# pypr/pysph

Hardware: AMD Instinct MI355X
Metric: particle-updates/sec (nnps.update + AccelerationEval.compute), WCSPH 3D, fp64 (higher is better)
Workload: dtype f64

## Files before the change

include/sphhip.h:

```cpp
#ifndef SPHHIP_H
#define SPHHIP_H

#include <stddef.h>
#include <stdint.h>

#ifdef __cplusplus
extern "C" {
#endif

#define SPH_MAX_ARRAYS 8
#define SPH_MAX_PAR 16
#define SPH_MAX_EQS 64

typedef struct sph_ctx sph_ctx;

enum sph_status {
    SPH_OK = 0,
    SPH_ERR_HIP = -1,
    SPH_ERR_ARG = -2,
    SPH_ERR_CELLS = -3,
    SPH_ERR_UNSUPPORTED = -4,
    SPH_ERR_MISSING_PROP = -5,
    SPH_ERR_STATE = -6
};
// ... 215 lines not shown
int sph_domain_counts_queue(sph_ctx *ctx);
int sph_domain_counts_collect(sph_ctx *ctx, double *out);
int sph_array_h_known(sph_ctx *ctx, int array_id, double *hmin, double *hmax);
int sph_array_props(sph_ctx *ctx, int array_id, int *out, int cap, int *n);
int sph_coord_histogram(sph_ctx *ctx, int array_id, int axis, double vmin, double span, int nbins, uint32_t *host_out);

enum sph_stepper {
    SPH_STEP_WCSPH = 1,
    SPH_STEP_TVF = 2,
    SPH_STEP_SOLID_MECH = 3
};
int sph_integrate_stage(sph_ctx *ctx, int array_id, int stepper, int stage, double dt);
int sph_reduce_min(sph_ctx *ctx, int array_id, int prop, double *out);

int sph_set_option(sph_ctx *ctx, const char *key, long value);

int sph_timer_enable(sph_ctx *ctx, int on);
int sph_timer_reset(sph_ctx *ctx);
int sph_timer_get(sph_ctx *ctx, const char *key, double *ms, long *count);

long sph_abi_sizeof(const char *struct_name);
long sph_abi_offsetof(const char *struct_name, const char *field);

#ifdef __cplusplus
}
#endif
#endif
```

pysph_amd/csrc/sph_eval.hip:

```cpp
#include "sph_internal.h"
#include "sph_kernels.h"
#include "sph_pair.h"

#include <cfloat>
#include <cmath>
#include <type_traits>

struct EosArgs {
    int kind;
    double par[SPH_MAX_PAR];
    double *rho, *p, *cs;
    size_t start, stop;
    double *q[SPH_PROP_COUNT];
    uint32_t *tflag;
};

__device__ inline void jacobi_eigen3(double A[3][3], double V[3][3], double d[3])
{
    for (int i = 0; i < 3; i++) for (int j = 0; j < 3; j++) V[i][j] = (i == j) ? 1.0 : 0.0;
    for (int sweep = 0; sweep < 12; sweep++) {
        double off = fabs(A[0][1]) + fabs(A[0][2]) + fabs(A[1][2]);
        double diag = fabs(A[0][0]) + fabs(A[1][1]) + fabs(A[2][2]);
        if (off <= 1e-300 || off <= 1e-18 * diag) break;
#pragma unroll
// ... 455 lines not shown
        if (a.dflags & F_MOM) {
            T au = D.au + a.p.gx, av = D.av + a.p.gy, aw = D.aw + a.p.gz;
            a.p.au[o] = au; a.p.av[o] = av; a.p.aw[o] = aw;
            a.p.dt_cfl[o] = D.dt_cfl < T(0.0) ? T(0.0) : D.dt_cfl + a.p.c0;
            a.p.dt_force[o] = au * au + av * av + aw * aw;
        }
        if (a.dflags & F_XSPH) {
            a.p.ax[o] = D.ax + D.u; a.p.ay[o] = D.ay + D.v; a.p.az[o] = D.az + D.w;
        }
    }
};
typedef FamWCSPH_T<double> FamWCSPH;

template <class T, bool UM = false> struct FamWCSPHE_T : FamWCSPH_T<T> {
    static constexpr bool EOSF = true;
    static constexpr bool UMASS = UM;
    static constexpr int NR = 8;
    struct Raw {
        typename std::conditional<sizeof(T) == 8, double2, float4>::type q[sizeof(T) == 8 ? 4 : 2];
    };
    template <class A> static __device__ __forceinline__ void load_raw(const A &a, uint32_t jg, Raw &r)
    {
        if constexpr (sizeof(T) == 8) {
            const double2 *p = reinterpret_cast<const double2 *>(a.rec) + (unsigned long long)jg * 4;
            r.q[0] = p[0]; r.q[1] = p[1]; r.q[2] = p[2]; r.q[3] = p[3];
        } else {
            const float4 *p = reinterpret_cast<const float4 *>(a.rec) + (unsigned long long)jg * 2;
            r.q[0] = p[0]; r.q[1] = p[1];
        }
    }
    template <class A> static __device__ __forceinline__ void decode(const A &a, const Raw &r, uint32_t fl, T mu, real4<T> &pj, T (&s)[8],
                                                                     int gk = 3)
    {
        T rho;
        if constexpr (sizeof(T) == 8) {
            pj.x = r.q[0].x; pj.y = r.q[0].y; pj.z = r.q[1].x; pj.w = 0.0;
            s[0] = r.q[1].y; s[1] = r.q[2].x; s[2] = r.q[2].y; s[3] = r.q[3].y; rho = r.q[3].x;
        } else {
            pj.x = r.q[0].x; pj.y = r.q[0].y; pj.z = r.q[0].z; pj.w = 0.f;
            s[0] = r.q[0].w; s[1] = r.q[1].x; s[2] = r.q[1].y; s[3] = r.q[1].w; rho = r.q[1].z;
        }
        s[4] = rho;
        s[5] = s[6] = s[7] = T(0.0);
        if constexpr (UM) {
            const T q = s[3];
            s[3] = mu;
            if (fl & F_MOM) {
                const T ratio = rho * (T)a.e_rho01;
                s[5] = q;
                s[6] = (T)a.e_c0 * tait_cs_power(ratio, gk);
// ... 14 lines not shown
        Raw r;
        load_raw(a, jg, r);
        decode(a, r, fl, mu, pj, s);
    }
};

template <class T, bool UM = false> struct FamWCSPHEG_T : FamWCSPHE_T<T, UM> {
    typedef FamWCSPHE_T<T, UM> Base;
    template <class A> static __device__ __forceinline__ void load_fused(const A &a, uint32_t jg, uint32_t fl, T mu, real4<T> &pj, T (&s)[8])
    {
        typename Base::Raw r;
        Base::load_raw(a, jg, r);
        Base::decode(a, r, fl, mu, pj, s, a.e_gk);
    }
};

template <class T> struct FamWCSPHV_T : FamWCSPH_T<T> {
    static constexpr bool EOSF = true;
    static constexpr int NR = 8;
    template <class A> static __device__ __forceinline__ void load_fused(const A &a, uint32_t jg, uint32_t fl, T mu, real4<T> &pj, T (&s)[8])
    {
        T rho;
        if constexpr (sizeof(T) == 8) {
            const double2 *p = reinterpret_cast<const double2 *>(a.rec) + (unsigned long long)jg * 4;
            const double2 q0 = p[0], q1 = p[1], q2 = p[2], q3 = p[3];
            pj.x = q0.x; pj.y = q0.y; pj.z = q1.x; pj.w = q1.y;
            s[0] = q2.x; s[1] = q2.y; s[2] = q3.x; rho = q3.y;
        } else {
            const float4 *p = reinterpret_cast<const float4 *>(a.rec) + (unsigned long long)jg * 2;
            const float4 q0 = p[0], q1 = p[1];
            pj.x = q0.x; pj.y = q0.y; pj.z = q0.z; pj.w = q0.w;
            s[0] = q1.x; s[1] = q1.y; s[2] = q1.z; rho = q1.w;
        }
        s[3] = mu;
        s[4] = rho;
        s[5] = s[6] = s[7] = T(0.0);
        if (fl & F_MOM) {
            const T ratio = rho * (T)a.e_rho01;
            T r7, r3;
            tait_powers(ratio, 3, r7, r3);
            const T p = (T)a.e_p0 + (T)a.e_B * (r7 - T(1.0));
            s[5] = rho != T(0.0) ? p * fast_rcp(rho * rho) : T(0.0);
            s[6] = (T)a.e_c0 * r3;
            s[7] = p;
        }
    }
};

#define WCSPHM_CT(f00, f01, f10, f11) ((uint32_t)(f00) | ((uint32_t)(f01) << 4) | ((uint32_t)(f10) << 8) | ((uint32_t)(f11) << 12))
template <class T> struct FamWCSPHM_T : FamWCSPHE_T<T, true> {
    typedef FamWCSPHE_T<T, true> Base;
    typedef typename Base::Raw Raw;
// ... 85 lines not shown
        const uint32_t ct = a.dflags;
        const uint32_t row = D.dc ? ((ct >> 8) | (ct >> 12)) & 15u : (ct | (ct >> 4)) & 15u;
        const size_t base = __builtin_offsetof(A, p) + __builtin_offsetof(Params, out) + (size_t)slot * (9 * sizeof(double *));
        auto out = [&](int k) { return kernarg_read<double *>(base + (size_t)k * sizeof(double *)); };
        if (row & F_CONT) out(0)[o] = D.arho;
        if (row & F_MOM) {
            const T au = D.au + a.p.gx, av = D.av + a.p.gy, aw = D.aw + a.p.gz;
            out(1)[o] = au; out(2)[o] = av; out(3)[o] = aw;
            out(7)[o] = D.dt_cfl < T(0.0) ? T(0.0) : D.dt_cfl + a.p.c0;
            out(8)[o] = au * au + av * av + aw * aw;
        }
        if (row & F_XSPH) {
            out(4)[o] = D.ax + D.u; out(5)[o] = D.ay + D.v; out(6)[o] = D.az + D.w;
        }
    }
};

template <class T> struct FamWCSPHMV_T : FamWCSPHM_T<T> {
    typedef FamWCSPHM_T<T> Base;
    template <class A> static __device__ __forceinline__ void load_fused(const A &a, uint32_t jg, uint32_t, T mu, real4<T> &pj, T (&s)[8])
    {
        T rho;
        if constexpr (sizeof(T) == 8) {
            const double2 *p = reinterpret_cast<const double2 *>(a.rec) + (unsigned long long)jg * 4;
            const double2 q0 = p[0], q1 = p[1], q2 = p[2], q3 = p[3];
            pj.x = q0.x; pj.y = q0.y; pj.z = q1.x; pj.w = q1.y;
            s[0] = q2.x; s[1] = q2.y; s[2] = q3.x; rho = q3.y;
        } else {
            const float4 *p = reinterpret_cast<const float4 *>(a.rec) + (unsigned long long)jg * 2;
            const float4 q0 = p[0], q1 = p[1];
            pj.x = q0.x; pj.y = q0.y; pj.z = q0.z; pj.w = q0.w;
            s[0] = q1.x; s[1] = q1.y; s[2] = q1.z; rho = q1.w;
        }
        const bool c1 = rho < T(0.0);
        s[3] = c1 ? -(T)a.p.mu1 : mu;
        rho = fabs(rho);
        s[4] = rho;
        const T ratio = rho * (T)a.e_rho01;
        T r7, r3;
        tait_powers(ratio, 3, r7, r3);
        const T p = (T)a.e_p0 + (T)a.e_B * (r7 - T(1.0));
        s[5] = rho != T(0.0) ? p * fast_rcp(rho * rho) : T(0.0);
        s[6] = (T)a.e_c0 * r3;
        s[7] = T(0.0);
    }
};

template <bool UH>
__device__ __forceinline__ void load_record_wcsph(const double *__restrict__ rj, uint32_t fl, double4 &pj, double (&s)[8])
{
    const double2 *r2 = reinterpret_cast<const double2 *>(rj);
    const double2 a0 = r2[0], a1 = r2[1], b0 = r2[2], b1 = r2[3], c = r2[4];
// ... 163 lines not shown
typedef FamTVF_T<double> FamTVF;

template <> __device__ __forceinline__ void load_record<FamTVF, true>(const double *__restrict__ rj, uint32_t fl, double4 &pj, double (&s)[12])
{
    const double2 *r2 = reinterpret_cast<const double2 *>(rj);
    const double2 a0 = r2[0], a1 = r2[1], b0 = r2[2], b1 = r2[3], c0 = r2[4];
    pj.x = a0.x; pj.y = a0.y; pj.z = a1.x; pj.w = 0.0;
    s[0] = b0.x; s[1] = b0.y; s[2] = b1.x; s[6] = a1.y; s[7] = b1.y; s[8] = 0.0; s[9] = 0.0; s[10] = c0.x; s[11] = 0.0;
    s[3] = s[4] = 0.0; s[5] = c0.y;
    if (fl & F_TAS) {
        const double2 d0 = r2[5];
        s[3] = d0.x; s[4] = d0.y;
    }
    if (fl & F_TAV) s[9] = r2[6].x;
}

template <class T> struct FamTVFE_T : FamTVF_T<T> {
    static constexpr bool EOSF = true;
    static constexpr int NA = 12;
    template <class A> static __device__ __forceinline__ void load_fused(const A &a, uint32_t jg, uint32_t fl, T mu, real4<T> &pj, T (&s)[12])
    {
        T rho;
        if constexpr (sizeof(T) == 8) {
            const double2 *p = reinterpret_cast<const double2 *>(a.rec) + (unsigned long long)jg * (unsigned)(a.nrec >> 1);
            const double2 q0 = p[0], q1 = p[1], q2 = p[2], q3 = p[3];
            pj.x = q0.x; pj.y = q0.y; pj.z = q1.x; pj.w = 0.0; rho = q1.y;
            s[0] = q2.x; s[1] = q2.y; s[2] = q3.x; s[3] = q3.y; s[4] = s[5] = 0.0;
            if (fl & F_TAS) { const double2 q4 = p[4]; s[4] = q4.x; s[5] = q4.y; }
        } else {
            const float4 *p = reinterpret_cast<const float4 *>(a.rec) + (unsigned long long)jg * (unsigned)(a.nrec >> 2);
            const float4 q0 = p[0], q1 = p[1];
            pj.x = q0.x; pj.y = q0.y; pj.z = q0.z; pj.w = 0.f; rho = q0.w;
            s[0] = q1.x; s[1] = q1.y; s[2] = q1.z; s[3] = q1.w; s[4] = s[5] = 0.f;
            if (fl & F_TAS) { const float4 q2 = p[2]; s[4] = q2.x; s[5] = q2.y; }
        }
        s[6] = rho;
        s[7] = (T)a.e_p0 * (rho * (T)a.e_rho01 - (T)a.e_B);
        s[8] = T(0.0);
        s[9] = mu;
        const T vj = mu * fast_rcp(rho);
        s[10] = vj * vj;
        s[11] = T(0.0);
    }
};

template <class T> struct FamVGrad_T {
    typedef T Real;
    static constexpr bool PRED = true;
    static constexpr uint32_t CF0 = F_VG3;
    static constexpr int MINB = 4;
    static constexpr int NA = 4;
    static constexpr int NR = 8;
    struct Params { double *v[9]; };
// ... 143 lines not shown
#pragma unroll
            for (int k = 0; k < 7; k++) q[k] = p[k];
            if (with_r) { q[7] = p[7]; q[8] = p[8]; q[9] = p[9]; }
            else q[7] = q[8] = q[9] = make_double2(0.0, 0.0);
            pj.x = q[0].x; pj.y = q[0].y; pj.z = q[1].x; pj.w = 0.0;
            s[0] = q[1].y; s[1] = q[2].x; s[2] = q[2].y; s[3] = mu; s[4] = q[3].x; s[5] = q[3].y;
#pragma unroll
            for (int k = 0; k < 6; k++) { s[6 + 2 * k] = q[4 + k].x; s[7 + 2 * k] = q[4 + k].y; }
        } else {
            float4 q[5];
#pragma unroll
            for (int k = 0; k < 4; k++) q[k] = p[k];
            if (with_r) q[4] = p[4];
            else { q[4] = make_float4(0.f, 0.f, 0.f, 0.f); q[3].z = 0.f; q[3].w = 0.f; }
            pj.x = q[0].x; pj.y = q[0].y; pj.z = q[0].z; pj.w = 0.f;
            s[0] = q[0].w; s[1] = q[1].x; s[2] = q[1].y; s[3] = mu; s[4] = q[1].z; s[5] = q[1].w;
#pragma unroll
            for (int k = 0; k < 3; k++) { s[6 + 4 * k] = q[2 + k].x; s[7 + 4 * k] = q[2 + k].y; s[8 + 4 * k] = q[2 + k].z; s[9 + 4 * k] = q[2 + k].w; }
        }
    }
    template <class A> static __device__ __forceinline__ void load_fused(const A &a, uint32_t jg, uint32_t, T mu, real4<T> &pj, T (&s)[18],
                                                                         uint32_t with_r = 1u)
    {
        decode(reinterpret_cast<const Piece *>(a.rec) + (unsigned long long)jg * PIECES, mu, pj, s, with_r);
    }
};

template <class Fam> __device__ __forceinline__ void load_aux(double (&s)[Fam::NA], const double *__restrict__ p)
{
#pragma unroll
    for (int k = 0; k < Fam::NA; k++) s[k] = p[k];
}

template <class Fam, int KK, bool UH> __global__ __launch_bounds__(256) void k_pair_direct(PairArgs<Fam> a)
{
    uint32_t i = blockIdx.x * blockDim.x + threadIdx.x;
    if (i >= a.nd) return;
    uint32_t o = a.d_perm[i];
    if (o < a.d_start || o >= a.d_stop) return;
    double4 pi = a.posh[a.d_off + i];
    typename Fam::Dest D;
    Fam::load(D, a.aux + (size_t)(a.d_off + i) * Fam::NA, a, o);
    uint32_t key = a.d_keys[i];
    int cx = key % a.nc[0];
    int t = key / a.nc[0];
    int cy = t % a.nc[1], cz = t / a.nc[1];
    double hi2 = a.radius_scale * pi.w;
// ... 166 lines not shown
        if (prop == SPH_M || prop == SPH_U || prop == SPH_V || prop == SPH_W) return true;
        if (prop == SPH_RHO) return flags & (F_MOM | F_XSPH);
        if (prop == SPH_P || prop == SPH_CS) return flags & F_MOM;
        return false;
    }
    if (fam == FAM_DENSITY) return prop == SPH_M;
    if (fam == FAM_NBR) return false;
    if (fam == FAM_VGRAD) return true;
    if (fam == FAM_ELASTIC) {
        if (prop == SPH_U || prop == SPH_V || prop == SPH_W || prop == SPH_M) return true;
        if (prop == SPH_RHO) return flags & (F_ESTRESS | F_EAV | F_EXSPH);
        if (prop == SPH_CS) return flags & F_EAV;
        if (prop == SPH_P) return flags & F_ESTRESS;
        if (prop >= SPH_S00 && prop <= SPH_S22) return flags & F_ESTRESS;
        return false;
    }
    if (fam == FAM_TVF) {
        if (prop == SPH_UHAT || prop == SPH_VHAT || prop == SPH_WHAT) return flags & F_TAS;
        return true;
    }
    return false;
}

static int pack_pieces(const PackArgs &pa)
{
    if (!pa.rec) return 0;
    if (pa.layout == 6) return 4;
    if (pa.layout == 7) return 2;
    if (pa.layout == 8) return pa.nr / 2;
    if (pa.layout == 9) return pa.nr / 4;
    if (pa.layout == 10) return 10;
    if (pa.layout == 11) return 5;
    if (pa.layout == 12) return 4;
    if (pa.layout == 13) return 2;
    if (pa.layout == 5) return (pa.nr % 4) ? 0 : pa.nr / 4;
    if (pa.nr % 2) return 0;
    return pa.nr / 2;
}

static void launch_pack(sph_ctx *c, const PackArgs &pa, size_t n)
{
    const dim3 g(div_up(n, 256)), b(256);
    const size_t lds = (size_t)pa.lds_np * 256 * 16;
    switch (pa.rec ? pa.layout : -1) {
    case 2: hipLaunchKernelGGL(k_pack<2>, g, b, lds, c->stream, pa); break;
    case 3: hipLaunchKernelGGL(k_pack<3>, g, b, lds, c->stream, pa); break;
// ... 207 lines not shown
    return SPH_OK;
}

int nnps_csr_pair_kernel(sph_ctx *c, int src, int dst, uint32_t *count, const uint32_t *start, uint32_t *nbrs)
{
    SPH_TRY(nnps_need_tables(c));
    DevArray &S = c->arr[src], &D = c->arr[dst];
    if (D.n == 0) return SPH_OK;
    if (count && D.n > D.n_binned) HIP_TRY(hipMemsetAsync(count + D.n_binned, 0, (D.n - D.n_binned) * 4, c->stream));
    const bool uh = c->uniform_h && c->use_uniform_h;
    const bool dest_is_src = src == dst;
    const size_t total = S.n + (dest_is_src ? 0 : D.n);
    if (total >= (1ull << 32)) { sph_set_error("too many particles for 32-bit packed indices"); return SPH_ERR_ARG; }
    PackPlan pl = pack_plan(FAM_NBR);
    if (uh) pl.nr = 4;
    const bool was_f32 = c->record_f32 != 0, was_a32 = c->arith_f32 != 0;
    c->record_f32 = 0; c->arith_f32 = 0;
    c->cur_eosf = false;
    c->cur_eosv = false;
    c->cur_tvff = false;
    c->cur_elu = false;
    c->cur_umass = false;
    c->cur_nrec = pl.nr;
    int rc = c->posh.reserve((total + 64) * sizeof(double) * pl.nr);
    if (rc == SPH_OK) rc = c->aux.reserve(64);
    if (rc == SPH_OK) rc = c->fposb.reserve((total + 64) * sizeof(float4));
    for (auto &pc : c->pack_cache) pc.epoch = 0;
    if (rc == SPH_OK) rc = pack_array(c, src, 0, pl, FAM_NBR, 1u, false, true, 0);
    if (rc == SPH_OK && S.g_n > 0) rc = pack_array(c, src, 0, pl, FAM_NBR, 1u, false, true, 1);
    if (rc == SPH_OK && !dest_is_src) rc = pack_array(c, dst, S.n, pl, FAM_NBR, 1u, true, true, 0);
    c->record_f32 = was_f32; c->arith_f32 = was_a32;
    if (rc != SPH_OK) return rc;
    sph_kernel K;
    K.kind = 1; K.dim = c->dim; K.fac = 1.0; K.radius_scale = c->radius_scale; K.deltap = 0.0;
    PairArgs<FamNbr> a;
    memset(&a, 0, sizeof a);
    fill_common(c, a, &K, 0.0);
    a.ablate = 0; a.dbg = nullptr;
    a.nsrc = 1;
    a.src[0] = {S.cell_start.as<uint32_t>(), 0u, 1u, S.fine_start.as<uint32_t>(), 0.0, 0u};
    if (S.g_n > 0) a.src[a.nsrc++] = {S.g_cell_start.as<uint32_t>(), (uint32_t)S.n_binned, 1u, S.g_fine_start.as<uint32_t>(), 0.0, 1u};
    a.d_off = dest_is_src ? 0u : (uint32_t)S.n;
    a.nd = (uint32_t)D.n_binned;
    a.d_keys = D.keys_sorted.as<uint32_t>(); a.d_fkeys = D.fkeys_sorted.as<uint32_t>(); a.d_perm = D.perm.as<uint32_t>();
    set_tile_order(c, a, D);
    a.d_start = 0; a.d_stop = (uint32_t)D.n; a.dflags = 1u;
    a.p.count = count; a.p.start = start; a.p.nbrs = nbrs;
// ... 82 lines not shown
        if (!A.m_known) return SPH_OK;
        if (have[cls[a]] && mu[cls[a]] != A.m_value) return SPH_OK;
        mu[cls[a]] = A.m_value; have[cls[a]] = true;
    }
    DevArray &M = c->merged;
    if (M.n == 0) { *done = true; return SPH_OK; }

    static const int outp[9] = {SPH_ARHO, SPH_AU, SPH_AV, SPH_AW, SPH_AX, SPH_AY, SPH_AZ, SPH_DT_CFL, SPH_DT_FORCE};
    static const int inp[9] = {SPH_X, SPH_Y, SPH_Z, SPH_U, SPH_V, SPH_W, SPH_RHO, SPH_P, SPH_H};
    const bool f32 = c->arith_f32 != 0;
    PackMArgs pa;
    memset(&pa, 0, sizeof pa);
    for (int a = 0; a < na; a++) {
        const int id = c->ids[a];
        DevArray &A = c->arr[id];
        for (int k = 0; k < 9; k++) {
            if (A.n && !A.prop[inp[k]]) return need_prop(c, id, inp[k], "pair loop");
            pa.prop[k][a] = A.prop[inp[k]];
        }
        if (cls[a]) pa.cls |= 1u << a;
    }
    c->cur_eosf = !vh; c->cur_umass = !vh; c->cur_tvff = false; c->cur_elu = false; c->cur_eosv = vh;
    c->cur_nrec = 8;
    SPH_TRY(c->posh.reserve((M.n + 64) * (f32 ? 32 : 64)));
    SPH_TRY(c->aux.reserve(64));
    SPH_TRY(c->fposb.reserve((M.n + 64) * sizeof(float4)));
    for (auto &pc : c->pack_cache) pc.epoch = 0;
    {
        ScopedTimer tm(c, T_PACK);
        pa.perm = M.perm.as<uint32_t>(); pa.slot = M.slot8.as<uint8_t>();
        pa.n = M.n; pa.off = 0;
        pa.rec = c->posh.as<double>(); pa.fpos = c->fposb.as<float4>();
        pa.f32 = f32 ? 1 : 0; pa.lds_np = f32 ? 2 : 4;
        for (int k = 0; k < 3; k++) pa.gmin[k] = c->xmin[k];
        pa.vh = vh ? 1 : 0;
        pa.hr = vh ? c->radius_scale : c->radius_scale * c->h_uniform;
        pa.rho_flag = c->xflag.as<uint32_t>();
        const dim3 pg(div_up(M.n, 256)), pb(256);
        const size_t plds = (size_t)pa.lds_np * 256 * 16;
        if (f32 && vh) hipLaunchKernelGGL((k_pack_merged<true, true>), pg, pb, plds, c->stream, pa);
        else if (f32) hipLaunchKernelGGL((k_pack_merged<true, false>), pg, pb, plds, c->stream, pa);
        else if (vh) hipLaunchKernelGGL((k_pack_merged<false, true>), pg, pb, plds, c->stream, pa);
        else hipLaunchKernelGGL((k_pack_merged<false, false>), pg, pb, plds, c->stream, pa);
    }
    ScopedTimer tm(c, T_PAIR);
    ScopedTimer tmf(c, T_PAIR_FAM + FAM_WCSPH);
// ... 199 lines not shown
                    !(c->uniform_h && c->use_uniform_h) && !(dflags & F_TENSILE) && tait_gk(g->eos_par[2]) == 3 && g->eos_par[0] > 0.0 &&
                    !c->record_f32 && !c->wcsph_nr;
        if (eosv) c->want_mrange = true;
        for (int j = 0; j < nsrcs && eosv; j++) eosv = c->arr[srcs[j]].m_known;
        if (eosv) pl.nr = 8;
        c->cur_eosv = eosv;
        bool tvff = g->src_eos == 2 && c->eos_fuse && c->mass_fuse && fam == FAM_TVF && c->pair_variant == 6 && c->uniform_h &&
                    c->use_uniform_h && !c->record_f32 && g->eos_par[1] != 0.0;
        if (tvff) c->want_mrange = true;
        for (int j = 0; j < nsrcs && tvff; j++) tvff = c->arr[srcs[j]].m_known;
        if (tvff && !dest_is_src) tvff = D.m_known;
        if (tvff) pl.nr = c->arith_f32 ? ((dflags & F_TAS) ? 12 : 8) : ((dflags & F_TAS) ? 10 : 8);
        bool elu = fam == FAM_ELASTIC && c->mass_fuse && c->pair_variant == 6 && c->uniform_h && c->use_uniform_h && !c->record_f32;
        if (elu) c->want_mrange = true;
        for (int j = 0; j < nsrcs && elu; j++) elu = c->arr[srcs[j]].m_known;
        if (elu) pl.nr = 20;
        c->cur_elu = elu;
        c->cur_tvff = tvff;
        c->cur_umass = umass;
        c->cur_eosf = eosf;
        c->cur_nrec = pl.nr;
        const void *rec_was = c->posh.ptr, *fpos_was = c->fposb.ptr;
        const size_t total_res = phase == 1 ? std::max(total, D.cap) : total;
        SPH_TRY(c->posh.reserve((total_res + 64) * sizeof(double) * (c->pair_variant >= 2 ? pl.nr : 4), phase == 2, c->stream));
        SPH_TRY(c->aux.reserve((total_res + 64) * sizeof(double) * pl.na));
        if (c->pair_variant >= 3) SPH_TRY(c->fposb.reserve((total_res + 64) * sizeof(float4), phase == 2, c->stream));
        if (c->posh.ptr != rec_was || c->fposb.ptr != fpos_was)
            for (auto &pc : c->pack_cache) pc.epoch = 0;
        {
            ScopedTimer tm(c, T_PACK);
            const int sig = pl.nr * 32 + (c->record_f32 ? 1 : 0) + (c->arith_f32 ? 2 : 0) + (eosf ? 4 : 0) + (umass ? 8 : 0) + (tvff || elu || eosv ? 16 : 0);
            if (phase == 1) c->phase_sig = sig;
            const bool repack = phase == 2 && c->phase_sig != sig;
            bool keep = share;
            if (share)
                for (auto &pc : c->pack_cache)
                    if (pc.epoch == c->pack_epoch && (pc.fam != fam || pc.sig != sig)) keep = false;
            if (!keep)
                for (auto &pc : c->pack_cache) pc.epoch = 0;
            auto pack_once = [&](int id, size_t off, uint32_t fl, bool dest_only) -> int {
                PackCache &pc = c->pack_cache[id];
                const bool hit = share && pc.epoch == c->pack_epoch && pc.fam == fam && pc.sig == sig;
                if (phase != 2 || repack) SPH_TRY(pack_array(c, id, off, pl, fam, fl, dest_only, !hit, 0));
                if (phase != 1 && c->arr[id].g_n > 0) SPH_TRY(pack_array(c, id, off, pl, fam, fl, dest_only, !hit, 1));
                pc.epoch = share ? c->pack_epoch : 0; pc.fam = fam; pc.sig = sig;
                return SPH_OK;
// ... 324 lines not shown
            if (D.nnps_slot < 0) { sph_set_error("destination array %d is not part of the neighbour grid", dst); return SPH_ERR_STATE; }
            if (c->ghosts_binned) { sph_set_error("generated families do not read ghost segments (ghost split): use the plain exchange -> sph_nnps_update order"); return SPH_ERR_UNSUPPORTED; }
            SPH_TRY(nnps_need_tables(c));
            size_t total = 0, off_of[SPH_MAX_ARRAYS];
            bool dest_is_src = false;
            for (int jj = 0; jj < ns; jj++) {
                const int s = f->src[idx[jj]];
                if (c->arr[s].nnps_slot < 0) { sph_set_error("source array %d is not part of the neighbour grid", s); return SPH_ERR_STATE; }
                off_of[jj] = total; total += c->arr[s].n; dest_is_src |= s == dst;
            }
            size_t d_off = total;
            if (!dest_is_src) total += D.n;
            else for (int jj = 0; jj < ns; jj++) if (f->src[idx[jj]] == dst) d_off = off_of[jj];
            if (total >= (1ull << 32)) { sph_set_error("too many particles for 32-bit packed indices"); return SPH_ERR_ARG; }
            const int na = f->n_sprops;
            const bool compact = q.uniform_h != 0;
            const int na_fam = ((na + 1) & ~1) < 2 ? 2 : ((na + 1) & ~1);
            a32 = c->arith_f32 && f->launch_f32 != nullptr;
            const bool rf32 = c->record_f32 || a32;
            const int nr = rf32 ? ((4 + na_fam + 3) & ~3)
                         : compact ? ((3 + na + 1) & ~1) : 4 + ((na + 1) & ~1);
            const int layout = rf32 ? 5 : (compact ? 4 : 0);
            q.rec_f32 = rf32 ? 1 : 0;
            SPH_TRY(c->posh.reserve((total + 64) * sizeof(double) * nr));
            for (auto &pc : c->pack_cache) pc.epoch = 0;
            SPH_TRY(c->aux.reserve(64));
            SPH_TRY(c->fposb.reserve((total + 64) * sizeof(float4)));
            {
                ScopedTimer tm(c, T_PACK);
                for (int jj = 0; jj < ns; jj++) SPH_TRY(pack_generic(c, f->src[idx[jj]], off_of[jj], na, f->sprops, nr, layout));
                if (!dest_is_src) {
                    int have[SPH_GEN_MAX_SPROPS], nh = 0;
                    for (int k = 0; k < na; k++) if (D.prop[f->sprops[k]]) have[nh++] = f->sprops[k];
                    SPH_TRY(pack_generic(c, dst, d_off, nh == na ? na : 0, f->sprops, nr, layout));
                }
            }
            q.rec = c->posh.as<double>();
            q.nrec = nr;
            q.fpos = c->fposb.as<float4>();
            q.dom_extent = fmax(fmax(c->xmax[0] - c->xmin[0], c->xmax[1] - c->xmin[1]), c->xmax[2] - c->xmin[2]);
            for (int k = 0; k < 3; k++) { q.nc[k] = c->nc[k]; q.xmin[k] = c->xmin[k]; }
            q.cell_size = c->cell_size;
            q.radius_scale = c->radius_scale;
            q.hu = 0.5 * (c->h_uniform + c->h_uniform);
            q.h1u = 1.0 / q.hu;
            q.facu = K->fac * q.h1u;
// ... 90 lines not shown
```

pysph_amd/csrc/sph_pair.h:

```cpp
#pragma once

#include <hip/hip_runtime.h>
#include <cstdint>

#include "sphhip.h"
#include "sph_kernels.h"

template <class T> __device__ __forceinline__ T r2_exact(T dx, T dy, T dz)
{
#pragma clang fp contract(off)
    const T a = dx * dx, b = dy * dy, c = dz * dz;
    return (a + b) + c;
}

template <class T> struct Real4Of;
template <> struct Real4Of<double> { typedef double4 type; };
template <> struct Real4Of<float> { typedef float4 type; };
template <class T> using real4 = typename Real4Of<T>::type;


struct KernelConst {
    double sigma;
    double deltap;
    int dim;
// ... 173 lines not shown
    T gg = aa * y, hh = 0.5 * y;
    const T rr = fma(-hh, gg, 0.5);
    hh = fma(hh, rr, hh);
    const T t = hh + hh;
    g.rinv = t * P;
    g.rij = r2c * g.rinv;
    g.q = g.rij * g.h1;
    return t * g.rij;
}

template <int KK, bool UH, class T> __device__ __forceinline__ T pair_w(const PairGeomT<T> &g) { return SphKernel<KK>::template w<UH>(g.q) * g.fac; }
template <int KK, bool UH, class T> __device__ __forceinline__ T pair_gradh(const PairGeomT<T> &g, int dim)
{
    return -g.fac * g.h1 * (SphKernel<KK>::template dw<UH>(g.q) * g.q + SphKernel<KK>::template w<UH>(g.q) * (T)dim);
}
template <int KK, bool UH, class T> __device__ __forceinline__ T pair_gradfac(const PairGeomT<T> &g)
{
    T t;
    if (SphKernel<KK>::HAS_DWQ) t = SphKernel<KK>::template dwq<UH>(g.q) * (g.fac * g.h1 * g.h1);
    else t = SphKernel<KK>::template dw<UH>(g.q) * (g.fac * g.h1) * g.rinv;
    return g.rij > T(1e-12) ? t : T(0);
}

template <class Fam, bool UH>
__device__ __forceinline__ void load_record(const double *__restrict__ rj, uint32_t fl, double4 &pj, double (&s)[Fam::NA])
{
    pj = *reinterpret_cast<const double4 *>(rj);
#pragma unroll
    for (int k = 0; k < Fam::NA; k++) s[k] = rj[4 + k];
}

template <class Fam, class T>
__device__ __forceinline__ void load_record_f32(const float *__restrict__ rj, real4<T> &pj, T (&s)[Fam::NA])
{
    constexpr int NF = (4 + Fam::NA + 3) & ~3;
    float f[NF];
    const float4 *r4 = reinterpret_cast<const float4 *>(rj);
#pragma unroll
    for (int q = 0; q < NF / 4; q++) { const float4 t = r4[q]; f[4 * q] = t.x; f[4 * q + 1] = t.y; f[4 * q + 2] = t.z; f[4 * q + 3] = t.w; }
    pj.x = f[0]; pj.y = f[1]; pj.z = f[2]; pj.w = f[3];
#pragma unroll
    for (int k = 0; k < Fam::NA; k++) s[k] = f[4 + k];
}

template <int NA, class T>
__device__ __forceinline__ void pin_record(const real4<T> &pj, const T (&s)[NA])
// ... 38 lines not shown
#endif
#define WLQ SPH_WLQ
#define WCAP_UH SPH_WCAP_UH
#define WCAP_VH 136
#define WCSL 96
#define NLW (64 * (1 + 3 * WLQ))
#define NL_NONE 0xFFFFFFFFu
#define XWIN (SPH_NSUB + 1)

#ifndef WPB
#define WPB 1
#endif

template <class Fam, int KK, bool UH, bool F32 = false, uint32_t CF = 0>
__global__ __launch_bounds__(64 * WPB, Fam::MINB) void k_pair_wave(PairArgs<Fam> a)
{
    typedef typename Fam::Real T;
    static_assert(F32 || sizeof(T) == 8, "fp32 arithmetic reads fp32 records");
    const uint32_t NR = (uint32_t)a.nrec;
    constexpr int WCAP = UH ? WCAP_UH : WCAP_VH;
    constexpr int TS = WCAP + 8;
    __shared__ __attribute__((aligned(16))) float tile_[WPB][(UH ? 3 : 4) * TS];
    __shared__ unsigned short csl_[WPB][WCSL];
    __shared__ unsigned long long smask_[WPB][WLQ][64];
    __shared__ uint32_t sjb_[WPB][WLQ][64];
    const int wv = __builtin_amdgcn_readfirstlane((int)(threadIdx.x >> 6));
    float *const tile = tile_[wv];
    float *const tx = tile, *const ty = tile + TS, *const tz = tile + 2 * TS, *const tw = tile + (UH ? 0 : 3 * TS);
    unsigned short *const csl = csl_[wv];
    unsigned long long (*const smask)[64] = smask_[wv];
    uint32_t (*const sjb)[64] = sjb_[wv];

    const int t = threadIdx.x & 63;
    const uint32_t wt = xcd_tile(blockIdx.x, gridDim.x) * WPB + (uint32_t)wv;
    uint32_t dtile = wt >> 2;
    if (dtile * 256u >= a.nd) return;
    if (a.d_tile_order) dtile = a.d_tile_order[dtile];
    const uint32_t tbase = dtile * 256u + (wt & 3u) * 64u;
    const uint32_t i = tbase + t;
    if (tbase >= a.nd) return;
    const bool valid = i < a.nd;
    uint32_t ic = valid ? i : a.nd - 1;
    if (a.d_list) ic = a.d_list[ic];
    const uint32_t o = a.d_perm[ic];
    uint32_t slot = 0;
    bool active;
    if constexpr (fam_merged<Fam>::value) {
        slot = a.d_slot[ic];
        const unsigned long long rg = kernarg_read<unsigned long long>(__builtin_offsetof(PairArgs<Fam>, p) + Fam::rng_offset(slot));
        active = valid && o >= (uint32_t)rg && o < (uint32_t)(rg >> 32);
    } else {
        active = valid && o >= a.d_start && o < a.d_stop;
    }
    const uint32_t fkey = a.d_fkeys[ic];
    const uint32_t key = fkey / SPH_NSUB;
    const int ncx = a.nc[0], ncy = a.nc[1], ncz = a.nc[2];
    const int row = key / ncx;
    const int cx = (int)(key % ncx) * SPH_NSUB + (int)(fkey % SPH_NSUB);
    bool facew = true;
    if (a.face_mode != 0 || a.gfx_lo > -0x7fffffff || a.gfx_hi < 0x7fffffff) {
        int mn = active ? cx : 0x7fffffff, mx = active ? cx : -0x7fffffff;
#pragma unroll
        for (int o = 32; o > 0; o >>= 1) { mn = min(mn, __shfl_xor(mn, o, 64)); mx = max(mx, __shfl_xor(mx, o, 64)); }
        mn = __builtin_amdgcn_readfirstlane(mn); mx = __builtin_amdgcn_readfirstlane(mx);
        facew = mn <= mx && (mn - XWIN <= a.gfx_lo || mx + XWIN >= a.gfx_hi);
        if (mn > mx && !a.nl_mode) return;
        if (a.face_mode == 1 && facew) return;
        if (a.face_mode == 2 && !facew) return;
    }
    real4<T> pi;
    typename Fam::Dest D;
    uint32_t wtok = 0;
    if constexpr (fam_token<Fam>::value) wtok = Fam::wave_token(a);
    T cur_mu = (T)a.d_mu;
    auto fetch = [&](uint32_t jg, uint32_t flags, real4<T> &pj, T (&sj)[Fam::NA]) {
        if constexpr (fam_token<Fam>::value) Fam::load_fused(a, jg, flags, cur_mu, pj, sj, wtok);
        else if constexpr (fam_eosf<Fam>::value) Fam::load_fused(a, jg, flags, cur_mu, pj, sj);
        else if constexpr (F32) load_record_f32<Fam, T>(reinterpret_cast<const float *>(a.rec) + (unsigned long long)jg * NR, pj, sj);
        else load_record<Fam, UH>(a.rec + (unsigned long long)jg * NR, flags, pj, sj);
    };
    {
        T sd_[Fam::NA];
        fetch(a.d_off + ic, a.dflags, pi, sd_);
        if (UH) pi.w = (T)a.hu;
        if constexpr (fam_merged<Fam>::value) Fam::load(D, sd_, a, o, slot);
        else Fam::load(D, sd_, a, o);
    }
    const int nfx = ncx * SPH_NSUB;
    const T hi_r = (T)a.radius_scale * pi.w;
    const T hi2 = UH ? (T)a.hr2u : hi_r * hi_r;
    const int row_first = __builtin_amdgcn_readfirstlane(row), row_last = __builtin_amdgcn_readlane(row, 63);
    if (DBGC(a) && t == 0) atomicAdd(DBGC(a) + 2, 1ull);

    auto do_pair = [&](uint32_t jg, uint32_t flags) {
        real4<T> pj;
        T sj[Fam::NA];
        fetch(jg, flags, pj, sj);
        pin_record<Fam::NA, T>(pj, sj);
        T hj2 = hi2;
        if (!UH) { hj2 = (T)a.radius_scale * pj.w; hj2 *= hj2; }
        const T r2 = r2_exact<T>(pi.x - pj.x, pi.y - pj.y, pi.z - pj.z);
        if (((r2 < hi2) || (r2 < hj2)) && ABLATE(a) != 1) Fam::template pair<KK, UH>(D, pi, pj, r2, sj, flags, a);
    };

    int cq = 0;
    auto phase2 = [&](uint32_t flags) {
        unsigned long long m = 0;
        uint32_t jb = 0;
        int q = 0;
        if (cq > 0 && ABLATE(a) != 2) { m = smask[0][t]; jb = sjb[0][t]; }
        const uint32_t self = a.d_off + ic;
        if (__any(m != 0)) {
            if (DBGC(a) && t == 0) atomicAdd(DBGC(a) + 1, 1ull);
            do {
                if (DBGC(a) && t == 0) atomicAdd(DBGC(a), 1ull);
                const bool has = m != 0;
                uint32_t j = has ? jb + (uint32_t)__builtin_ctzll(m) : self;
                m &= m - 1;
                if (m == 0 && q + 1 < cq) { ++q; m = smask[q][t]; jb = sjb[q][t]; }
                if (ABLATE(a) == 3) j = self;
                if constexpr (Fam::PRED) {
                    real4<T> pj;
                    T sj[Fam::NA];
                    fetch(j, flags, pj, sj);
                    T hj2 = hi2;
                    if (!UH) { hj2 = (T)a.radius_scale * pj.w; hj2 *= hj2; }
                    const T r2 = r2_exact<T>(pi.x - pj.x, pi.y - pj.y, pi.z - pj.z);
                    const bool pass = has && ((r2 < hi2) || (r2 < hj2)) && ABLATE(a) != 1;
                    Fam::template pair<KK, UH>(D, pi, pj, r2, sj, flags, a, pass);
                } else {
                    if (has) do_pair(j, flags);
                }
            } while (__any(m != 0));
        }
        cq = 0;
    };

    uint32_t *const nlw = a.nl_mode ? a.nl + (size_t)wt * NLW : nullptr;
    bool reuse = false, unsaved = false;
    if (a.nl_mode == 2) {
        const uint32_t nq = nlw[t];
        reuse = !__any(nq == NL_NONE);
        if (reuse) {
            const uint32_t off0 = a.src[0].off;
            const int nqmax = wave_max_i32((int)nq);
            for (int q = 0; q < nqmax; q++) {
                const uint32_t *w = nlw + 64 * (1 + 3 * q) + t;
                smask[q][t] = (unsigned long long)w[0] | ((unsigned long long)w[64] << 32);
                sjb[q][t] = w[128] + off0;
            }
            __builtin_amdgcn_fence(__ATOMIC_ACQ_REL, "wavefront");
            cq = active ? (int)nq : 0;
        }
    }

    for (int s = 0; s < a.nsrc; s++) {
    const SrcDesc sd = a.src[s];
    if (sd.ghost && !facew) continue;
    const uint32_t fl = CF ? CF : sd.flags;
    cur_mu = (T)sd.mu;
    int R = row_first, st = 0, part_resume = 0;
    uint32_t tb_resume = 0;
    bool resumed = false;
    for (;;) {
    bool more = false;
    for (; R <= row_last && !more && !reuse && ABLATE(a) != 6; R++, st = 0) {
        const bool inseg = active && row == R;
        const unsigned long long segm = __ballot(inseg);
        if (!segm) continue;
        const int cxa = __builtin_amdgcn_readlane(cx, __builtin_ctzll(segm));
        const int cxb = __builtin_amdgcn_readlane(cx, 63 - __builtin_clzll(segm));
        const int cyR = R % ncy, czR = R / ncy;
        const int xa = max(cxa - XWIN, 0), xb = min(cxb + XWIN, nfx - 1);
        const int ncs = xb - xa + 2;
        const double binw = a.cell_size * (1.0 / SPH_NSUB);
// ... 79 lines not shown
                                d = __builtin_elementwise_fma(ez, ez, d);
                                mm = __builtin_amdgcn_alignbit(mm, __float_as_uint(d.x), 31);
                                mm = __builtin_amdgcn_alignbit(mm, __float_as_uint(d.y), 31);
                            }
                        }
                        if (g8 < 4) mm <<= 8 * (4 - g8);
                        mm = __builtin_bitreverse32(mm);
                        const int rem = lenc - 32 * gw;
                        wd[gw] = rem >= 32 ? mm : (rem > 0 ? (mm & ((1u << rem) - 1u)) : 0u);
                    }
                    unsigned long long m0 = (unsigned long long)wd[0] | ((unsigned long long)wd[1] << 32);
                    uint32_t m2 = wd[2];
                    uint32_t jb0 = sd.off + tb + (uint32_t)ps0;
                    if (a.norm_masks && __any(m2 != 0)) {
                        const int sh = m0 ? __builtin_ctzll(m0) : (m2 ? 64 + __builtin_ctz(m2) : 0);
                        if (sh >= 64) { m0 = (unsigned long long)(m2 >> (sh - 64)); m2 = 0; }
                        else if (sh > 0) {
                            m0 = (m0 >> sh) | ((unsigned long long)m2 << (64 - sh));
                            m2 = sh >= 32 ? 0u : (m2 >> sh);
                        }
                        jb0 += (uint32_t)sh;
                    }
                    if (__any(cq + (m0 != 0) + (m2 != 0) > WLQ)) { more = true; break; }
                    if (m0) { smask[cq][t] = m0; sjb[cq][t] = jb0; cq++; }
                    if (m2) { smask[cq][t] = m2; sjb[cq][t] = jb0 + 64u; cq++; }
                }
                __builtin_amdgcn_fence(__ATOMIC_ACQ_REL, "wavefront");
                if (more) { tb_resume = tb; part_resume = part; break; }
            }
            if (more) break;
        }
        if (more) break;
    }
    if (a.nl_mode == 1 && s == 0) {
        if (unsaved || more) nlw[t] = NL_NONE;
        else {
            __builtin_amdgcn_fence(__ATOMIC_ACQ_REL, "wavefront");
            nlw[t] = (uint32_t)cq;
            const int nqmax = wave_max_i32(cq);
            for (int q = 0; q < nqmax; q++) {
                uint32_t *w = nlw + 64 * (1 + 3 * q) + t;
                const unsigned long long m = q < cq ? smask[q][t] : 0ull;
                w[0] = (uint32_t)m; w[64] = (uint32_t)(m >> 32);
                w[128] = q < cq ? sjb[q][t] - sd.off : 0u;
            }
        }
    }
    phase2(fl);
    if (!more) break;
    unsaved = true;
    resumed = true;
    }
    }
    if (active) {
        if constexpr (fam_merged<Fam>::value) Fam::finish(D, a, o, slot);
        else Fam::finish(D, a, o);
    }
}


template <class F, class = void> struct fam_rowlds { static constexpr bool value = false; };
template <class F> struct fam_rowlds<F, decltype((void)F::ROWLDS)> { static constexpr bool value = F::ROWLDS; };

#ifndef SPH_WCAP_L
#define SPH_WCAP_L 96
#endif
#define WCAP_L SPH_WCAP_L

template <class Fam, int KK, uint32_t CF = 0>
__global__ __launch_bounds__(64, Fam::MINB) void k_pair_rowlds(PairArgs<Fam> a)
{
    typedef typename Fam::Real T;
    typedef typename Fam::Piece Piece;
    constexpr int NP = Fam::PIECES;
    constexpr int TS = WCAP_L + 8;
    static_assert(WCAP_L <= AMAXLEN && WCAP_L % 8 == 0, "one part per tile");
    __shared__ __attribute__((aligned(16))) float tile[3 * TS];
    __shared__ unsigned short csl[WCSL];
    __shared__ __attribute__((aligned(16))) Piece recs[WCAP_L * NP];
// ... 155 lines not shown
```

pysph_amd/device.py:

```python
import ctypes as C
import os

import numpy as np

from .particle_array import get_npy

_HERE = os.path.dirname(os.path.abspath(__file__))
LIB_PATH = os.environ.get('SPH_LIBRARY') or os.path.join(_HERE, 'libsphhip.so')

MAX_ARRAYS = 8
MAX_PAR = 16


class SphKernel(C.Structure):
    _fields_ = [('kind', C.c_int), ('dim', C.c_int), ('fac', C.c_double),
                ('radius_scale', C.c_double), ('deltap', C.c_double)]


class SphEquation(C.Structure):
    _fields_ = [('kind', C.c_int), ('dest', C.c_int), ('nsrc', C.c_int),
                ('src', C.c_int * MAX_ARRAYS), ('par', C.c_double * MAX_PAR)]


class SphGroup(C.Structure):
    _fields_ = [('real', C.c_int), ('start_idx', C.c_long),
                ('stop_idx', C.c_long), ('neq', C.c_int),
                ('eqs', C.POINTER(SphEquation)),
                ('src_eos', C.c_int), ('eos_par', C.c_double * 4),
                ('nl_mode', C.c_int), ('phase', C.c_int)]


_P = C.c_void_p
_PD = C.POINTER(C.c_double)
_PU = C.POINTER(C.c_uint32)
SIGNATURES = {
    'sph_abi_sizeof': (C.c_long, [C.c_char_p]),
    'sph_abi_offsetof': (C.c_long, [C.c_char_p, C.c_char_p]),
    'sph_ctx_create': (C.c_int, [C.c_int, _P, C.POINTER(_P)]),
    'sph_ctx_destroy': (C.c_int, [_P]),
    'sph_ctx_synchronize': (C.c_int, [_P]),
    'sph_last_error': (C.c_char_p, []),
    'sph_version': (C.c_char_p, []),
    'sph_prop_id': (C.c_int, [C.c_char_p]),
    'sph_array_resize': (C.c_int, [_P, C.c_int, C.c_size_t, C.c_size_t]),
    'sph_array_size': (C.c_int, [_P, C.c_int, C.POINTER(C.c_size_t),
                                 C.POINTER(C.c_size_t)]),
    'sph_array_ensure_prop': (C.c_int, [_P, C.c_int, C.c_int]),
    'sph_array_permute': (C.c_int, [_P, C.c_int, C.POINTER(C.c_uint32), C.c_size_t,
                                    C.c_size_t]),
    'sph_array_push': (C.c_int, [_P, C.c_int, C.c_int, _PD, C.c_size_t,
                                 C.c_size_t]),
    'sph_array_pull': (C.c_int, [_P, C.c_int, C.c_int, _PD, C.c_size_t,
                                 C.c_size_t]),
    'sph_array_device_ptr': (C.c_int, [_P, C.c_int, C.c_int, C.POINTER(_P)]),
    'sph_nnps_update': (C.c_int, [_P, C.c_int, C.c_int, C.POINTER(C.c_int),
                                  C.c_double, C.c_double, _PD]),
    'sph_nnps_info': (C.c_int, [_P, _PD, C.POINTER(C.c_long)]),
    'sph_nnps_minmax': (C.c_int, [_P, C.c_int, C.POINTER(C.c_int), _PD]),
    'sph_nnps_get_csr': (C.c_int, [_P, C.c_int, C.c_int, _PU, C.c_size_t, _PU,
                                   C.c_size_t, C.POINTER(C.c_size_t)]),
# ... 604 lines not shown
```

Measured before the change: 1.980 billion.

## Use 32-bit record offsets and a fixed-trip neighbour loop in pair kernel

Record addressing in the pair kernels switches from 64-bit index multiplication to 32-bit byte offsets via a rec_at helper. Host-side checks reject record buffers over 4 GiB. The phase-2 neighbour loop is restructured: masks are split into lo/hi 32-bit shared slots, and a per-lane hit count fixes the loop trip count at the wave maximum, replacing the data-dependent __any loop. The finish step reloads the output index through d_perm behind an opaque asm barrier, which is meant to cut register pressure and 64-bit address arithmetic but adds a load and relies on the 4 GiB limit.

Result: faster. 2.009 billion (median of 6 runs) (+1.4%).

```diff
diff --git a/include/sphhip.h b/include/sphhip.h
--- a/include/sphhip.h
+++ b/include/sphhip.h
@@ -261,6 +261,8 @@
 long sph_abi_sizeof(const char *struct_name);
 long sph_abi_offsetof(const char *struct_name, const char *field);
 
+int sph_check_record_bytes(size_t n_records, size_t rec_bytes);
+
 #ifdef __cplusplus
 }
 #endif
diff --git a/pysph_amd/csrc/sph_eval.hip b/pysph_amd/csrc/sph_eval.hip
--- a/pysph_amd/csrc/sph_eval.hip
+++ b/pysph_amd/csrc/sph_eval.hip
@@ -501,10 +501,10 @@
     template <class A> static __device__ __forceinline__ void load_raw(const A &a, uint32_t jg, Raw &r)
     {
         if constexpr (sizeof(T) == 8) {
-            const double2 *p = reinterpret_cast<const double2 *>(a.rec) + (unsigned long long)jg * 4;
+            const double2 *p = rec_at<double2>(a.rec, jg, 64u);
             r.q[0] = p[0]; r.q[1] = p[1]; r.q[2] = p[2]; r.q[3] = p[3];
         } else {
-            const float4 *p = reinterpret_cast<const float4 *>(a.rec) + (unsigned long long)jg * 2;
+            const float4 *p = rec_at<float4>(a.rec, jg, 32u);
             r.q[0] = p[0]; r.q[1] = p[1];
         }
     }
@@ -565,12 +565,12 @@
     {
         T rho;
         if constexpr (sizeof(T) == 8) {
-            const double2 *p = reinterpret_cast<const double2 *>(a.rec) + (unsigned long long)jg * 4;
+            const double2 *p = rec_at<double2>(a.rec, jg, 64u);
             const double2 q0 = p[0], q1 = p[1], q2 = p[2], q3 = p[3];
             pj.x = q0.x; pj.y = q0.y; pj.z = q1.x; pj.w = q1.y;
             s[0] = q2.x; s[1] = q2.y; s[2] = q3.x; rho = q3.y;
         } else {
-            const float4 *p = reinterpret_cast<const float4 *>(a.rec) + (unsigned long long)jg * 2;
+            const float4 *p = rec_at<float4>(a.rec, jg, 32u);
             const float4 q0 = p[0], q1 = p[1];
             pj.x = q0.x; pj.y = q0.y; pj.z = q0.z; pj.w = q0.w;
             s[0] = q1.x; s[1] = q1.y; s[2] = q1.z; rho = q1.w;
@@ -702,12 +702,12 @@
     {
         T rho;
         if constexpr (sizeof(T) == 8) {
-            const double2 *p = reinterpret_cast<const double2 *>(a.rec) + (unsigned long long)jg * 4;
+            const double2 *p = rec_at<double2>(a.rec, jg, 64u);
             const double2 q0 = p[0], q1 = p[1], q2 = p[2], q3 = p[3];
             pj.x = q0.x; pj.y = q0.y; pj.z = q1.x; pj.w = q1.y;
             s[0] = q2.x; s[1] = q2.y; s[2] = q3.x; rho = q3.y;
         } else {
-            const float4 *p = reinterpret_cast<const float4 *>(a.rec) + (unsigned long long)jg * 2;
+            const float4 *p = rec_at<float4>(a.rec, jg, 32u);
             const float4 q0 = p[0], q1 = p[1];
             pj.x = q0.x; pj.y = q0.y; pj.z = q0.z; pj.w = q0.w;
             s[0] = q1.x; s[1] = q1.y; s[2] = q1.z; rho = q1.w;
@@ -917,13 +917,13 @@
     {
         T rho;
         if constexpr (sizeof(T) == 8) {
-            const double2 *p = reinterpret_cast<const double2 *>(a.rec) + (unsigned long long)jg * (unsigned)(a.nrec >> 1);
+            const double2 *p = rec_at<double2>(a.rec, jg, ((uint32_t)a.nrec >> 1) * 16u);
             const double2 q0 = p[0], q1 = p[1], q2 = p[2], q3 = p[3];
             pj.x = q0.x; pj.y = q0.y; pj.z = q1.x; pj.w = 0.0; rho = q1.y;
             s[0] = q2.x; s[1] = q2.y; s[2] = q3.x; s[3] = q3.y; s[4] = s[5] = 0.0;
             if (fl & F_TAS) { const double2 q4 = p[4]; s[4] = q4.x; s[5] = q4.y; }
         } else {
-            const float4 *p = reinterpret_cast<const float4 *>(a.rec) + (unsigned long long)jg * (unsigned)(a.nrec >> 2);
+            const float4 *p = rec_at<float4>(a.rec, jg, ((uint32_t)a.nrec >> 2) * 16u);
             const float4 q0 = p[0], q1 = p[1];
             pj.x = q0.x; pj.y = q0.y; pj.z = q0.z; pj.w = 0.f; rho = q0.w;
             s[0] = q1.x; s[1] = q1.y; s[2] = q1.z; s[3] = q1.w; s[4] = s[5] = 0.f;
@@ -1113,7 +1113,7 @@
     template <class A> static __device__ __forceinline__ void load_fused(const A &a, uint32_t jg, uint32_t, T mu, real4<T> &pj, T (&s)[18],
                                                                          uint32_t with_r = 1u)
     {
-        decode(reinterpret_cast<const Piece *>(a.rec) + (unsigned long long)jg * PIECES, mu, pj, s, with_r);
+        decode(rec_at<Piece>(a.rec, jg, PIECES * (uint32_t)sizeof(Piece)), mu, pj, s, with_r);
     }
 };
 
@@ -1326,6 +1326,15 @@
     return false;
 }
 
+int sph_check_record_bytes(size_t n_records, size_t rec_bytes)
+{
+    const size_t lim = (size_t)1 << 32;
+    if (rec_bytes == 0 || n_records <= lim / rec_bytes) return SPH_OK;
+    sph_set_error("%zu records of %zu bytes need %.2f GiB: over the 4 GiB the pair kernels address with 32-bit record offsets",
+                  n_records, rec_bytes, (double)n_records * (double)rec_bytes / (double)lim);
+    return SPH_ERR_UNSUPPORTED;
+}
+
 static int pack_pieces(const PackArgs &pa)
 {
     if (!pa.rec) return 0;
@@ -1579,7 +1588,8 @@
     c->cur_elu = false;
     c->cur_umass = false;
     c->cur_nrec = pl.nr;
-    int rc = c->posh.reserve((total + 64) * sizeof(double) * pl.nr);
+    int rc = sph_check_record_bytes(total + 64, sizeof(double) * pl.nr);
+    if (rc == SPH_OK) rc = c->posh.reserve((total + 64) * sizeof(double) * pl.nr);
     if (rc == SPH_OK) rc = c->aux.reserve(64);
     if (rc == SPH_OK) rc = c->fposb.reserve((total + 64) * sizeof(float4));
     for (auto &pc : c->pack_cache) pc.epoch = 0;
@@ -1708,6 +1718,7 @@
     }
     c->cur_eosf = !vh; c->cur_umass = !vh; c->cur_tvff = false; c->cur_elu = false; c->cur_eosv = vh;
     c->cur_nrec = 8;
+    SPH_TRY(sph_check_record_bytes(M.n + 64, f32 ? 32 : 64));
     SPH_TRY(c->posh.reserve((M.n + 64) * (f32 ? 32 : 64)));
     SPH_TRY(c->aux.reserve(64));
     SPH_TRY(c->fposb.reserve((M.n + 64) * sizeof(float4)));
@@ -1953,6 +1964,7 @@
         c->cur_nrec = pl.nr;
         const void *rec_was = c->posh.ptr, *fpos_was = c->fposb.ptr;
         const size_t total_res = phase == 1 ? std::max(total, D.cap) : total;
+        SPH_TRY(sph_check_record_bytes(total_res + 64, sizeof(double) * (c->pair_variant >= 2 ? pl.nr : 4)));
         SPH_TRY(c->posh.reserve((total_res + 64) * sizeof(double) * (c->pair_variant >= 2 ? pl.nr : 4), phase == 2, c->stream));
         SPH_TRY(c->aux.reserve((total_res + 64) * sizeof(double) * pl.na));
         if (c->pair_variant >= 3) SPH_TRY(c->fposb.reserve((total_res + 64) * sizeof(float4), phase == 2, c->stream));
@@ -2323,6 +2335,7 @@
                          : compact ? ((3 + na + 1) & ~1) : 4 + ((na + 1) & ~1);
             const int layout = rf32 ? 5 : (compact ? 4 : 0);
             q.rec_f32 = rf32 ? 1 : 0;
+            SPH_TRY(sph_check_record_bytes(total + 64, sizeof(double) * nr));
             SPH_TRY(c->posh.reserve((total + 64) * sizeof(double) * nr));
             for (auto &pc : c->pack_cache) pc.epoch = 0;
             SPH_TRY(c->aux.reserve(64));
diff --git a/pysph_amd/csrc/sph_pair.h b/pysph_amd/csrc/sph_pair.h
--- a/pysph_amd/csrc/sph_pair.h
+++ b/pysph_amd/csrc/sph_pair.h
@@ -219,6 +219,11 @@
     return g.rij > T(1e-12) ? t : T(0);
 }
 
+template <class P> __device__ __forceinline__ const P *rec_at(const void *base, uint32_t jg, uint32_t bytes)
+{
+    return reinterpret_cast<const P *>(reinterpret_cast<const char *>(base) + jg * bytes);
+}
+
 template <class Fam, bool UH>
 __device__ __forceinline__ void load_record(const double *__restrict__ rj, uint32_t fl, double4 &pj, double (&s)[Fam::NA])
 {
@@ -303,16 +308,16 @@
     constexpr int TS = WCAP + 8;
     __shared__ __attribute__((aligned(16))) float tile_[WPB][(UH ? 3 : 4) * TS];
     __shared__ unsigned short csl_[WPB][WCSL];
-    __shared__ unsigned long long smask_[WPB][WLQ][64];
-    __shared__ uint32_t sjb_[WPB][WLQ][64];
+    __shared__ uint32_t slots_[WPB][3][WLQ][64];
     const int wv = __builtin_amdgcn_readfirstlane((int)(threadIdx.x >> 6));
     float *const tile = tile_[wv];
     float *const tx = tile, *const ty = tile + TS, *const tz = tile + 2 * TS, *const tw = tile + (UH ? 0 : 3 * TS);
     unsigned short *const csl = csl_[wv];
-    unsigned long long (*const smask)[64] = smask_[wv];
-    uint32_t (*const sjb)[64] = sjb_[wv];
+    uint32_t (*const smlo)[64] = slots_[wv][0], (*const smhi)[64] = slots_[wv][1], (*const sjb)[64] = slots_[wv][2];
 
     const int t = threadIdx.x & 63;
+    auto put_slot = [&](int q, unsigned long long m, uint32_t jb) { smlo[q][t] = (uint32_t)m; smhi[q][t] = (uint32_t)(m >> 32); sjb[q][t] = jb; };
+    auto slot_mask = [&](int q) { return (unsigned long long)smlo[q][t] | ((unsigned long long)smhi[q][t] << 32); };
     const uint32_t wt = xcd_tile(blockIdx.x, gridDim.x) * WPB + (uint32_t)wv;
     uint32_t dtile = wt >> 2;
     if (dtile * 256u >= a.nd) return;
@@ -357,8 +362,8 @@
     auto fetch = [&](uint32_t jg, uint32_t flags, real4<T> &pj, T (&sj)[Fam::NA]) {
         if constexpr (fam_token<Fam>::value) Fam::load_fused(a, jg, flags, cur_mu, pj, sj, wtok);
         else if constexpr (fam_eosf<Fam>::value) Fam::load_fused(a, jg, flags, cur_mu, pj, sj);
-        else if constexpr (F32) load_record_f32<Fam, T>(reinterpret_cast<const float *>(a.rec) + (unsigned long long)jg * NR, pj, sj);
-        else load_record<Fam, UH>(a.rec + (unsigned long long)jg * NR, flags, pj, sj);
+        else if constexpr (F32) load_record_f32<Fam, T>(rec_at<float>(a.rec, jg, NR * 4u), pj, sj);
+        else load_record<Fam, UH>(rec_at<double>(a.rec, jg, NR * 8u), flags, pj, sj);
     };
     {
         T sd_[Fam::NA];
@@ -385,36 +390,41 @@
     };
 
     int cq = 0;
+    uint32_t nh = 0;
     auto phase2 = [&](uint32_t flags) {
-        unsigned long long m = 0;
-        uint32_t jb = 0;
-        int q = 0;
-        if (cq > 0 && ABLATE(a) != 2) { m = smask[0][t]; jb = sjb[0][t]; }
         const uint32_t self = a.d_off + ic;
-        if (__any(m != 0)) {
-            if (DBGC(a) && t == 0) atomicAdd(DBGC(a) + 1, 1ull);
-            do {
-                if (DBGC(a) && t == 0) atomicAdd(DBGC(a), 1ull);
-                const bool has = m != 0;
-                uint32_t j = has ? jb + (uint32_t)__builtin_ctzll(m) : self;
-                m &= m - 1;
-                if (m == 0 && q + 1 < cq) { ++q; m = smask[q][t]; jb = sjb[q][t]; }
-                if (ABLATE(a) == 3) j = self;
-                if constexpr (Fam::PRED) {
-                    real4<T> pj;
-                    T sj[Fam::NA];
-                    fetch(j, flags, pj, sj);
-                    T hj2 = hi2;
-                    if (!UH) { hj2 = (T)a.radius_scale * pj.w; hj2 *= hj2; }
-                    const T r2 = r2_exact<T>(pi.x - pj.x, pi.y - pj.y, pi.z - pj.z);
-                    const bool pass = has && ((r2 < hi2) || (r2 < hj2)) && ABLATE(a) != 1;
-                    Fam::template pair<KK, UH>(D, pi, pj, r2, sj, flags, a, pass);
-                } else {
-                    if (has) do_pair(j, flags);
-                }
-            } while (__any(m != 0));
+        if (cq == 0) put_slot(0, 1ull, self);
+        const uint32_t qlast = cq > 0 ? (uint32_t)cq - 1u : 0u;
+        const int kmax = ABLATE(a) == 2 ? 0 : wave_max_i32((int)nh);
+        unsigned long long m = slot_mask(0);
+        uint32_t jb = sjb[0][t], q = 0;
+        if (DBGC(a) && kmax > 0 && t == 0) atomicAdd(DBGC(a) + 1, 1ull);
+        for (int k = 0; k < kmax; k++) {
+            if (DBGC(a) && t == 0) atomicAdd(DBGC(a), 1ull);
+            const bool has = (uint32_t)k < nh;
+            uint32_t j = jb + (uint32_t)__builtin_ctzll(m);
+            m &= m - 1;
+            const bool step = m == 0;
+            q = min(q + (uint32_t)step, qlast);
+            const unsigned long long mn = slot_mask((int)q);
+            jb = sjb[q][t];
+            m = step ? mn : m;
+            if (ABLATE(a) == 3) j = self;
+            if constexpr (Fam::PRED) {
+                real4<T> pj;
+                T sj[Fam::NA];
+                fetch(j, flags, pj, sj);
+                T hj2 = hi2;
+                if (!UH) { hj2 = (T)a.radius_scale * pj.w; hj2 *= hj2; }
+                const T r2 = r2_exact<T>(pi.x - pj.x, pi.y - pj.y, pi.z - pj.z);
+                const bool pass = has && ((r2 < hi2) || (r2 < hj2)) && ABLATE(a) != 1;
+                Fam::template pair<KK, UH>(D, pi, pj, r2, sj, flags, a, pass);
+            } else {
+                if (has) do_pair(j, flags);
+            }
         }
         cq = 0;
+        nh = 0;
     };
 
     uint32_t *const nlw = a.nl_mode ? a.nl + (size_t)wt * NLW : nullptr;
@@ -425,13 +435,14 @@
         if (reuse) {
             const uint32_t off0 = a.src[0].off;
             const int nqmax = wave_max_i32((int)nq);
+            cq = active ? (int)nq : 0;
             for (int q = 0; q < nqmax; q++) {
                 const uint32_t *w = nlw + 64 * (1 + 3 * q) + t;
-                smask[q][t] = (unsigned long long)w[0] | ((unsigned long long)w[64] << 32);
-                sjb[q][t] = w[128] + off0;
+                const unsigned long long m = (unsigned long long)w[0] | ((unsigned long long)w[64] << 32);
+                put_slot(q, m, w[128] + off0);
+                if (q < cq) nh += (uint32_t)__builtin_popcountll(m);
             }
             __builtin_amdgcn_fence(__ATOMIC_ACQ_REL, "wavefront");
-            cq = active ? (int)nq : 0;
         }
     }
 
@@ -557,8 +568,9 @@
                         jb0 += (uint32_t)sh;
                     }
                     if (__any(cq + (m0 != 0) + (m2 != 0) > WLQ)) { more = true; break; }
-                    if (m0) { smask[cq][t] = m0; sjb[cq][t] = jb0; cq++; }
-                    if (m2) { smask[cq][t] = m2; sjb[cq][t] = jb0 + 64u; cq++; }
+                    if (m0) { put_slot(cq, m0, jb0); cq++; }
+                    if (m2) { put_slot(cq, m2, jb0 + 64u); cq++; }
+                    nh += (uint32_t)(__builtin_popcountll(m0) + __builtin_popcount(m2));
                 }
                 __builtin_amdgcn_fence(__ATOMIC_ACQ_REL, "wavefront");
                 if (more) { tb_resume = tb; part_resume = part; break; }
@@ -575,7 +587,7 @@
             const int nqmax = wave_max_i32(cq);
             for (int q = 0; q < nqmax; q++) {
                 uint32_t *w = nlw + 64 * (1 + 3 * q) + t;
-                const unsigned long long m = q < cq ? smask[q][t] : 0ull;
+                const unsigned long long m = q < cq ? slot_mask(q) : 0ull;
                 w[0] = (uint32_t)m; w[64] = (uint32_t)(m >> 32);
                 w[128] = q < cq ? sjb[q][t] - sd.off : 0u;
             }
@@ -588,8 +600,11 @@
     }
     }
     if (active) {
-        if constexpr (fam_merged<Fam>::value) Fam::finish(D, a, o, slot);
-        else Fam::finish(D, a, o);
+        uint32_t icf = ic;
+        asm volatile("" : "+v"(icf));
+        const uint32_t of = *rec_at<uint32_t>(a.d_perm, icf, 4u);
+        if constexpr (fam_merged<Fam>::value) Fam::finish(D, a, of, slot);
+        else Fam::finish(D, a, of);
     }
 }
 
diff --git a/pysph_amd/device.py b/pysph_amd/device.py
--- a/pysph_amd/device.py
+++ b/pysph_amd/device.py
@@ -36,6 +36,7 @@
 SIGNATURES = {
     'sph_abi_sizeof': (C.c_long, [C.c_char_p]),
     'sph_abi_offsetof': (C.c_long, [C.c_char_p, C.c_char_p]),
+    'sph_check_record_bytes': (C.c_int, [C.c_size_t, C.c_size_t]),
     'sph_ctx_create': (C.c_int, [C.c_int, _P, C.POINTER(_P)]),
     'sph_ctx_destroy': (C.c_int, [_P]),
     'sph_ctx_synchronize': (C.c_int, [_P]),
```
